# LouisRouss/DiffuLab

Hardware: AMD Instinct MI355X
Metric: train images/sec/node (DiT-S/2 flow-matching, 256x256 latents) (higher is better)
Workload: dtype bf16

## Files before the change

diffulab_amd/csrc/embed.hip:

```cpp
#include "common.h"
#include "aux_paths.h"
#include <atomic>

static std::atomic<int> g_last_aux_path{DL_AUX_PATH_NONE};
void dl_note_aux_path(int path) { g_last_aux_path.store(path, std::memory_order_relaxed); }
extern "C" __attribute__((visibility("default"))) int dl_lab_last_aux_path() { return g_last_aux_path.load(std::memory_order_relaxed); }

__global__ void patchify_k(const float* __restrict__ x, bf16_t* __restrict__ tok, int B, int C, int H, int W, int p,
                           int ld, int order) {
  const int gh = H / p, gw = W / p, F = C * p * p;
  const int64_t total = (int64_t)B * gh * gw * ld, stride = (int64_t)gridDim.x * blockDim.x;
  for (int64_t i = (int64_t)blockIdx.x * blockDim.x + threadIdx.x; i < total; i += stride) {
    const int f = (int)(i % ld);
    const int64_t t = i / ld;
    float val = 0.f;
    if (f < F) {
      const int wq = (int)(t % gw), hq = (int)((t / gw) % gh), b = (int)(t / ((int64_t)gw * gh));
      int c, p1, p2;
      if (order == DL_PATCH_CPP) {
        p2 = f % p;
        p1 = (f / p) % p;
        c = f / (p * p);
      } else {
        c = f % C;
// ... 148 lines not shown
                                     dl_stream_t stream) {
  DL_CHECK_ARG(t && out && B > 0 && dim > 0 && dim % 2 == 0, "dl_timestep_embedding: dim must be even");
  const int half = (int)(dim / 2);
  int64_t g = (B * half + 255) / 256;
  if (g > 1024) g = 1024;
  hipLaunchKernelGGL(timestep_embedding_k, (int)g, 256, 0, (hipStream_t)stream, t, (bf16_t*)out, (int)B, (int)dim,
                     (float)(-log((double)max_period) / (double)half));
  DL_LAUNCH_CHECK();
  return DL_OK;
}

__global__ void cond_combine_fwd_k(const float* __restrict__ e, const float* __restrict__ table,
                                   const int64_t* __restrict__ idx, float* __restrict__ emb, bf16_t* __restrict__ act,
                                   int B, int E) {
  const int64_t total = (int64_t)B * E;
  for (int64_t i = (int64_t)blockIdx.x * blockDim.x + threadIdx.x; i < total; i += (int64_t)gridDim.x * blockDim.x) {
    const int b = (int)(i / E), c = (int)(i % E);
    float v = e[i];
    if (idx) v += table[idx[b] * E + c];
    emb[i] = v;
    act[i] = f2bf(silu_f(v));
  }
}
extern "C" int dl_cond_combine_fwd(const float* e, const float* table, const int64_t* idx, float* emb, void* act,
                                   int64_t B, int64_t E, dl_stream_t stream) {
  DL_CHECK_ARG(e && emb && act && B > 0 && E > 0 && (!idx || table), "dl_cond_combine_fwd: bad args");
  int64_t g = (B * E + 255) / 256;
  if (g > 1024) g = 1024;
  hipLaunchKernelGGL(cond_combine_fwd_k, (int)g, 256, 0, (hipStream_t)stream, e, table, idx, emb, (bf16_t*)act, (int)B,
                     (int)E);
  DL_LAUNCH_CHECK();
  return DL_OK;
}
__global__ void cond_combine_bwd_k(const float* __restrict__ dact, const float* __restrict__ emb,
                                   const int64_t* __restrict__ idx, float* __restrict__ demb,
                                   bf16_t* __restrict__ demb16, float* __restrict__ dtable, int B, int E) {
  const int64_t total = (int64_t)B * E;
  for (int64_t i = (int64_t)blockIdx.x * blockDim.x + threadIdx.x; i < total; i += (int64_t)gridDim.x * blockDim.x) {
    const int b = (int)(i / E), c = (int)(i % E);
    const float g = dact[i] * dsilu_f(emb[i]);
    demb[i] = g;
    if (demb16) demb16[i] = f2bf(g);
    if (dtable && idx) {
      const int64_t lab = idx[b];
      bool first = true;
      for (int b2 = 0; b2 < b; ++b2) first = first && idx[b2] != lab;
      if (first) {
        float acc = g;
        for (int b2 = b + 1; b2 < B; ++b2)
          if (idx[b2] == lab) acc += dact[(int64_t)b2 * E + c] * dsilu_f(emb[(int64_t)b2 * E + c]);
        dtable[lab * E + c] += acc;
      }
    }
  }
}
extern "C" int dl_cond_combine_bwd(const float* dact, const float* emb, const int64_t* idx, float* demb, void* demb_bf16,
                                   float* dtable, int64_t B, int64_t E, dl_stream_t stream) {
  DL_CHECK_ARG(dact && emb && demb && B > 0 && E > 0, "dl_cond_combine_bwd: bad args");
  int64_t g = (B * E + 255) / 256;
  if (g > 1024) g = 1024;
  hipLaunchKernelGGL(cond_combine_bwd_k, (int)g, 256, 0, (hipStream_t)stream, dact, emb, idx, demb, (bf16_t*)demb_bf16,
                     dtable, (int)B, (int)E);
  DL_LAUNCH_CHECK();
  return DL_OK;
}

__global__ void cond_combine_dense_fwd_k(const float* __restrict__ e, const float* __restrict__ pe, float* __restrict__ emb,
                                         bf16_t* __restrict__ act, int64_t n4) {
  for (int64_t i = (int64_t)blockIdx.x * blockDim.x + threadIdx.x; i < n4; i += (int64_t)gridDim.x * blockDim.x) {
    const float4 a = ((const float4*)e)[i], p = ((const float4*)pe)[i];
    const float4 v = make_float4(a.x + p.x, a.y + p.y, a.z + p.z, a.w + p.w);
    ((float4*)emb)[i] = v;
    ((uint2*)act)[i] = make_uint2((uint32_t)f2bf(silu_f(v.x)) | ((uint32_t)f2bf(silu_f(v.y)) << 16),
                                  (uint32_t)f2bf(silu_f(v.z)) | ((uint32_t)f2bf(silu_f(v.w)) << 16));
  }
}
extern "C" int dl_cond_combine_dense_fwd(const float* e, const float* pe, float* emb, void* act, int64_t B, int64_t E,
                                         dl_stream_t stream) {
  DL_CHECK_ARG(e && pe && emb && act && B > 0 && E > 0 && E % 4 == 0 && ((uintptr_t)e | (uintptr_t)pe | (uintptr_t)emb) % 16 == 0 &&
                   (uintptr_t)act % 8 == 0,
               "dl_cond_combine_dense_fwd: contiguous [B, E] operands, E a multiple of 4 (E=%lld), f32 operands 16-byte, act 8-byte aligned",
               (long long)E);
  const int64_t n4 = B * E / 4;
  int64_t g = (n4 + 255) / 256;
  if (g > 1024) g = 1024;
  hipLaunchKernelGGL(cond_combine_dense_fwd_k, (int)g, 256, 0, (hipStream_t)stream, e, pe, emb, (bf16_t*)act, n4);
  DL_LAUNCH_CHECK();
  return DL_OK;
}
__global__ void cond_combine_dense_bwd_k(const float* __restrict__ dact, const float* __restrict__ emb, float* __restrict__ demb,
                                         bf16_t* __restrict__ demb16, int64_t n4) {
  for (int64_t i = (int64_t)blockIdx.x * blockDim.x + threadIdx.x; i < n4; i += (int64_t)gridDim.x * blockDim.x) {
    const float4 d = ((const float4*)dact)[i], v = ((const float4*)emb)[i];
    const float4 g = make_float4(d.x * dsilu_f(v.x), d.y * dsilu_f(v.y), d.z * dsilu_f(v.z), d.w * dsilu_f(v.w));
    ((float4*)demb)[i] = g;
// ... 459 lines not shown
```

diffulab_amd/engine.py:

```python

from __future__ import annotations

import functools
import math
from dataclasses import dataclass, field

import torch
from torch import Tensor

from . import ops, tuning


_PARAM_EPOCH = 0


def bump_param_epoch() -> None:
    global _PARAM_EPOCH
    _PARAM_EPOCH += 1


def _must(ok: bool) -> None:
    if not ok:
        raise RuntimeError("a HIP kernel declined a shape the engine had selected it for")


def _rup(x: int, m: int) -> int:
    return (x + m - 1) // m * m


STREAMS = ("input", "context")
ROW_MAX_DIM = 4096
F32_MAX_DIM = 1024


@functools.lru_cache(maxsize=None)
def block_names(pre: str, st: str | None = None) -> dict[str, str]:
    if st is None:
        n = dict(n1="norm_1", n2="norm_2", qk="attention.qk_norm", qkv="attention.qkv", proj="attention.proj_out", up="mlp_input.0",
                 down="mlp_input.2")
    else:
        n = dict(n1=f"{st}_norm_1", n2=f"{st}_norm_2", qk=f"attention.qk_norm_{st}", qkv=f"attention.qkv_{st}",
                 proj=f"attention.{st}_proj_out", up=f"mlp_{st}.0", down=f"mlp_{st}.2")
    return {k: pre + v for k, v in n.items()}


@dataclass(slots=True)
class Modulation:
    mat: Tensor
    dmat: Tensor | None
    off: int
    D: int
    rows: int
    tok: bool = False
    part: Tensor | tuple | None = None
    groups: int = 0

    def col(self, c: int) -> Tensor:
        o = self.off + c * self.D
        return self.mat[:, o : o + self.D]

# ... 474 lines not shown
        B, _, _, _, _, _, M, _, _ = self.geo
        D, E = d.inner_dim, d.embedding_dim
        ops.patchify(x, w["tokP"], d.patch_size, ops.PATCH_CPP)
        if patch_gemm:
            ops.gemm_nt(w["tokP"], sh[self._conv_name + "|f"], w["x"][0] if x0 is None else x0, M=M, N=D, K=self._ki)
        ops.timestep_embedding(t, w["temb"][:B])
        ops.gemm_nt(w["temb"], sh["time_embed.0.weight|f"], w["h1"], bias=self.P("time_embed.0.bias"), act=ops.ACT_SILU,
                    pre_out=w["pre1"], M=B, N=E, K=d.frequency_embedding)
        ops.gemm_nt(w["h1"], sh["time_embed.2.weight|f"], w["e"], bias=self.P("time_embed.2.bias"), M=B, N=E, K=E)
        if self._pooled_dim:
            self._pooled_fwd(B)
        else:
            table = self.P("label_embed.embedding.weight") if d.n_classes is not None else None
            ops.cond_combine_fwd(w["e"][:B], table, y_eff if table is not None else None, w["emb"][:B], w["se"][:B])
        mod_bias = self.params[self.layout.entries[self.layout.mod_b0][0] :][: self.layout.mod_rows]
        ops.gemm_nt(w["se"], sh["@mod|f"], w["mod"], bias=mod_bias, M=B, N=self.layout.mod_rows, K=E)
        return w["mod"]

    def _pooled_fwd(self, B: int) -> None:
        d, w, sh = self.d, self.ws, self.sh
        E, P = d.embedding_dim, self._pooled_dim
        pooled = self.pooled
        assert pooled is not None and tuple(pooled.shape) == (B, P), "pooled context embedding [B, pooled_dim] not set for this step"
        w["poolP"][:B, :P].copy_(pooled)
        ops.gemm_nt(w["poolP"], sh["mlp_pooled_context.0.weight|f"], w["ph1"], bias=self.P("mlp_pooled_context.0.bias"), act=ops.ACT_SILU,
                    pre_out=w["ppre1"], M=B, N=2 * E, K=w["poolP"].shape[1])
        ops.gemm_nt(w["ph1"], sh["mlp_pooled_context.2.weight|f"], w["pe"], bias=self.P("mlp_pooled_context.2.bias"), M=B, N=E, K=2 * E)
        ops.cond_combine_dense_fwd(w["e"][:B], w["pe"][:B], w["emb"][:B], w["se"][:B])

    def _pooled_bwd(self, B: int, det: Tensor | None) -> None:
        d, w, sh = self.d, self.ws, self.sh
        E, P = d.embedding_dim, self._pooled_dim
        ops.colsum(w["demb"], self.G("mlp_pooled_context.2.bias"), B, E, scratch=det)
        ops.gemm_tn(w["demb16"], w["ph1"], self.G("mlp_pooled_context.2.weight"), scratch=det)
        ops.gemm_nt(w["demb16"], sh["mlp_pooled_context.2.weight|t"], w["dph1"], M=B, N=2 * E, K=E)
        ops.silu_bwd(w["dph1"][:B], w["ppre1"][:B], w["dppre1"][:B])
        ops.gemm_tn(w["dppre1"], w["poolP"], self.G("mlp_pooled_context.0.weight"), M=2 * E, N=P, scratch=det)
        ops.colsum(w["dppre1"], self.G("mlp_pooled_context.0.bias"), B, 2 * E, scratch=det)

    def _main_wgs(self) -> int:
        explicit = tuning.integer("DL_MAIN_WGS", 0)
        if explicit:
            return explicit
        reserve = tuning.integer("DL_DP_RESERVE_CUS", 0)
        if reserve and self.reducer is not None and getattr(self.reducer, "enabled", True):
            if getattr(self, "_cus", None) is None:
                self._cus = torch.cuda.get_device_properties(self.dev).multi_processor_count
            return max(8, (self._cus - reserve) & ~7)
        return 0

    def _native_blocks(self) -> bool:
        return type(self) is DiTEngine and tuning.on("DL_NATIVE_BLOCK") and not (self.geo is not None and ops.attn_needs_padding(self.geo[5]))

    def _block_args(self, i: int, train: bool):
        key = (self._ws_key, i, self.reducer is None, self._main_wgs())
        blk = self._blk_cache.get(key)
        if blk is not None:
            return blk
        from ._block import DitBlock

        d, w, sh = self.d, self.ws, self.sh
        B, _, _, gh, gw, N, M, Bp, Fo = self.geo
        D, L, F = d.inner_dim, d.depth, d.mlp_ratio * d.inner_dim
        pre, mo = f"layers.{i}.", i * 6 * D
        mod, xs = w["mod"], w["x"]
        a = w["layers"][i if train else 0]
        xin = xs[i] if train else xs[i & 1]
        cos, sin = self._rope[(gh, gw)]
        mrow = lambda off: mod.data_ptr() + 2 * off
        blk = DitBlock()
        blk.B, blk.N, blk.D, blk.H, blk.F = B, N, D, d.num_heads, F
# ... 513 lines not shown
        _must(ops.ln_modulate_gemm_bwd(g["du"], sh[nm["up"] + ".weight|t"], a["x1"], self.P(nm["n2"] + ".weight"),
                                        self.P(nm["n2"] + ".bias"), mod[:, mo + 3 * D : mo + 4 * D], N, a["mean2"], a["rstd2"], dx, nx,
                                        dmod[:, mo + 3 * D : mo + 4 * D], dmod[:, mo + 4 * D : mo + 5 * D], w["dwb"][2 * i + 1],
                                        gate_t=a["t1"], gate=mod[:, mo + 2 * D : mo + 3 * D], dt=g["dt1"],
                                        dgate=dmod[:, mo + 2 * D : mo + 3 * D]))
        if fold:
            sw.fold(w["dwb"][2 * i + 1], nm["n2"] + ".weight", self.geo[0])
        dx = nx
        sw.wgrad(g["dt1"], a["a"], nm["proj"] + ".weight")
        ops.gemm_nt(g["dt1"], sh[nm["proj"] + ".weight|t"], s["da"])
        self._attn_bwd(a, g, nm, s, N, *self._rope[(gh, gw)], None, None, None)
        sw.wgrad(g["dqkv"], a["xm1"], nm["qkv"] + ".weight")
        if dres is not None:
            ops.add_bf16(dx, dres, dx)
        nxt = {}
        if i > 0:
            mp = (i - 1) * 6 * D
            nxt = dict(gate_t=w["layers"][i - 1]["t2"], gate=mod[:, mp + 5 * D : mp + 6 * D], dt=w["wg"][i - 1]["dt2"],
                       dgate=dmod[:, mp + 5 * D : mp + 6 * D])
        nx = _other(s, dx)
        _must(ops.ln_modulate_gemm_bwd(g["dqkv"], sh[nm["qkv"] + ".weight|t"], w["x"][i], self.P(nm["n1"] + ".weight"),
                                        self.P(nm["n1"] + ".bias"), mod[:, mo : mo + D], N, a["mean1"], a["rstd1"], dx, nx,
                                        dmod[:, mo : mo + D], dmod[:, mo + D : mo + 2 * D], w["dwb"][2 * i], **nxt))
        if fold:
            sw.fold(w["dwb"][2 * i], nm["n1"] + ".weight", self.geo[0])
        return nx

    def _head_bwd(self, dpred: Tensor, dxm: Tensor | None, scratch: Tensor | None = None) -> None:
        d, w = self.d, self.ws
        M, Fo, D = self.geo[6], self.geo[8], d.inner_dim
        ops.patchify(dpred, w["dO"], d.patch_size, ops.PATCH_PPC)
        gl = self.G("last_layer.linear.weight")
        if Fo % 8 == 0:
            ops.gemm_tn(w["dO"], w["xf"], gl, M=Fo, N=D, scratch=scratch)
        else:
            w["scr_last"].zero_()
            ops.gemm_tn(w["dO"], w["xf"], w["scr_last"], M=_rup(Fo, 8), N=D, scratch=scratch)
            ops.reduce_rows_f32(w["scr_last"], gl, 1, Fo * D)
        ops.colsum(w["dO"], self.G("last_layer.linear.bias"), M, Fo, scratch=scratch)
        if dxm is not None:
            ops.gemm_nt(w["dO"], self.sh["last_layer.linear.weight|t"], dxm, M=M, N=D, K=self._ko)

    def _dfeat_rows(self, dfeats: dict[int, Tensor] | None) -> dict[int, Tensor]:
        return {k: g.reshape(-1, self.d.inner_dim).to(torch.bfloat16).contiguous() for k, g in (dfeats or {}).items()}

    def _patch_wgrad(self, dx: Tensor, name: str, scratch: Tensor | None) -> None:
        d, w = self.d, self.ws
        D, Fi = d.inner_dim, d.input_channels * d.patch_size**2
        gc = self.G(name).view(D, Fi)
        if Fi % 8 == 0:
            ops.gemm_tn(dx, w["tokP"], gc, M=D, N=Fi, scratch=scratch)
        else:
            w["scr_conv"].zero_()
            ops.gemm_tn(dx, w["tokP"], w["scr_conv"], M=D, N=_rup(Fi, 8), scratch=scratch)
            gc.add_(w["scr_conv"][:, :Fi])

    def _end_block(self, sw: "SideWork", bi: int) -> None:
        sw.flush()
        if self.reducer is not None:
            self.reducer.ready(*self.layer_ranges[bi], extra_events=(sw.side.record_event(),))

    def _cond_bwd(self, dx: Tensor, extra_demb: Tensor | None = None) -> None:
        d, w, sh = self.d, self.ws, self.sh
        B, _, _, _, _, _, M, _, _ = self.geo
        D, E = d.inner_dim, d.embedding_dim
        dmod = w["dmod32"]
        det = w.get("det_scr")
        self._patch_wgrad(dx, self._conv_name, det)

        R = self.layout.mod_rows
        g_modw = self.grads[self.layout.entries[self.mod_name][0] :][: R * E].view(R, E)
        g_modb = self.grads[self.layout.entries[self.layout.mod_b0][0] :][:R]
        L6 = len(self.prefixes) * 6 * D if getattr(self, "_early_mod_done", False) else 0
        if L6:
            ops.cast2d_f32_to_bf16(dmod[:B, L6:], w["dmod"][:B, L6:])
            dmod = w["dmod"]
            ops.gemm_tn(dmod[:, L6:], w["se"], g_modw[L6:], scratch=det)
            ops.colsum(dmod[:, L6:], g_modb[L6:], B, R - L6, scratch=det)
        else:
            ops.cast_f32_to_bf16(dmod[:B], w["dmod"][:B])
            dmod = w["dmod"]
            ops.gemm_tn(dmod, w["se"], g_modw, scratch=det)
            ops.colsum(dmod, g_modb, B, R, scratch=det)
        ops.gemm_nt(dmod, sh["@mod|t"], w["dse"], M=B, N=E, K=R, scratch=det)
        table = d.n_classes is not None
        if self._pooled_dim:
            ops.cond_combine_dense_bwd(w["dse"][:B], w["emb"][:B], w["demb"][:B], w["demb16"][:B])
            self._pooled_bwd(B, det)
        else:
            ops.cond_combine_bwd(w["dse"][:B], w["emb"][:B], self._yeff if table else None, w["demb"][:B], w["demb16"][:B],
                                 self.G("label_embed.embedding.weight") if table else None)
        if extra_demb is not None:
            w["demb"][:B].add_(extra_demb[:B])
            ops.cast_f32_to_bf16(w["demb"][:B], w["demb16"][:B])
        ops.colsum(w["demb"], self.G("time_embed.2.bias"), B, E, scratch=det)
        ops.gemm_tn(w["demb16"], w["h1"], self.G("time_embed.2.weight"), scratch=det)
        ops.gemm_nt(w["demb16"], sh["time_embed.2.weight|t"], w["dh1"], M=B, N=E, K=E)
        ops.silu_bwd(w["dh1"][:B], w["pre1"][:B], w["dpre1"][:B])
        ops.gemm_tn(w["dpre1"], w["temb"], self.G("time_embed.0.weight"), scratch=det)
        ops.colsum(w["dpre1"], self.G("time_embed.0.bias"), B, E, scratch=det)
        if self.reducer is not None:
            if L6:
                w_mod = self.layout.entries[self.mod_name][0]
                self.reducer.ready(0, w_mod)
                self.reducer.ready(w_mod + L6 * E, self.layer_ranges[0][0])
            else:
                self.reducer.ready(0, self.layer_ranges[0][0])
            self.reducer.finish()


class _StrictWgradGroups(ops.WgradGroups):

    def _issue(self, key: int) -> None:
        probs = self.pending.pop(key, [])
        if probs:
            self.launch(lambda: _must(ops.gemm_tn_group(probs, self.slab, max_wgs=self.max_wgs)))


class _NoSideWork:

    def wgrad(self, dy: Tensor, x: Tensor, name: str) -> None:
        pass

    def fold(self, partial: Tensor | None, name: str, groups: int) -> None:
        pass

    def flush(self) -> None:
        pass

    def join(self) -> None:
        pass


# ... 35 lines not shown
```

diffulab_amd/ops.py:

```python

from __future__ import annotations

import ctypes
import os

import torch
from torch import Tensor

from ._lib import lib
from . import tuning

BF16, F32 = 0, 1
ACT_NONE, ACT_SILU, ACT_GELU = 0, 1, 2
LOSS_FLOW, LOSS_EPS = 0, 1
MEAN_TYPES = {"epsilon": 0, "xstart": 1, "xprev": 2, "v": 3}
VAR_MODES = {"learned": 0, "learned_range": 1}
VAR_FIXED = -1
PATCH_CPP, PATCH_PPC = 0, 1


_raw_stream = getattr(torch._C, "_cuda_getCurrentRawStream", None)


def _s() -> int:
# ... 539 lines not shown
    gemm_nt(dt, w2t, dh)
    swiglu_bwd(dh, u, du)


def mlp_dswiglu_recompute(x: Tensor, wp: Tensor, dt: Tensor, w2t: Tensor, du: Tensor) -> bool:
    M, F = x.shape[0], w2t.shape[0]
    return _maybe("dl_mlp_dswiglu_recompute", _p(x), x.stride(0), _p(wp), wp.stride(0), _p(dt), dt.stride(0), _p(w2t), w2t.stride(0),
                  _p(du), du.stride(0), M, F, x.shape[1], dt.shape[1], _s())


def _padded_rows(t: Tensor) -> Tensor:
    base = t._base
    if base is not None and base.dim() == t.dim() and base.shape[1:] == t.shape[1:] and base.data_ptr() == t.data_ptr() \
            and base.shape[0] == (t.shape[0] + 63) // 64 * 64 and base.stride() == t.stride():
        return base
    return t


def gemm_tn(a: Tensor, b: Tensor, out: Tensor, *, M: int | None = None, N: int | None = None, max_wgs: int = 0,
            scratch: Tensor | None = None) -> Tensor:
    M = a.shape[1] if M is None else M
    N = b.shape[1] if N is None else N
    if a.shape[0] % 64:
        a, b = _padded_rows(a), _padded_rows(b)
        assert a.shape[0] == b.shape[0], "gemm_tn operands with a ragged row count must be zero-padded row buffers"
    if scratch is not None:
        _call("dl_gemm_tn_det", _p(a), a.stride(0), _p(b), b.stride(0), _p(out), out.stride(0), M, N, a.shape[0], _p(scratch),
              scratch.numel(), _s())
        return out
    _call("dl_gemm_tn_ex", _p(a), a.stride(0), _p(b), b.stride(0), _p(out), out.stride(0), M, N, a.shape[0], int(max_wgs), _s())
    return out


class _WGrad(ctypes.Structure):

    _fields_ = [("dy", ctypes.c_void_p), ("ld_dy", ctypes.c_int64), ("x", ctypes.c_void_p), ("ld_x", ctypes.c_int64),
                ("g", ctypes.c_void_p), ("m_out", ctypes.c_int64), ("n_in", ctypes.c_int64)]


def gemm_tn_group(probs: list[tuple[Tensor, Tensor, Tensor]], slab: Tensor, max_wgs: int = 0) -> bool:
    arr = (_WGrad * len(probs))()
    if probs[0][0].shape[0] % 64:
        probs = [(_padded_rows(dy), _padded_rows(x), g) for dy, x, g in probs]
    R = probs[0][0].shape[0]
    for q, (dy, x, g) in zip(arr, probs):
        assert dy.shape[0] == R and x.shape[0] == R and g.is_contiguous()
        q.dy, q.ld_dy, q.x, q.ld_x, q.g, q.m_out, q.n_in = _p(dy), dy.stride(0), _p(x), x.stride(0), _p(g), g.shape[0], g.shape[1]
    global _LIB
    if _LIB is None:
        _LIB = lib()
    fn = _LIB._fns["dl_gemm_tn_group"][0]
    rc = fn(ctypes.addressof(arr), len(probs), R, _p(slab), slab.numel(), int(max_wgs), _s())
    if rc == -3:
        return False
    if rc != 0:
        raise RuntimeError(f"dl_gemm_tn_group failed ({rc}): {_LIB.cdll.dl_last_error().decode()}")
    return True


_SCRATCH: dict = {}


def shared_scratch(device, floats: int) -> Tensor:
    key = (torch.device(device).type, torch.device(device).index)
    buf = _SCRATCH.get(key)
    if buf is None or buf.numel() < floats:
# ... 980 lines not shown
```

diffulab_amd/tuning.py:

```python

from __future__ import annotations

import os

SWITCHES: dict[str, tuple[str, str]] = {
    "DL_NATIVE_BLOCK": ("1", "DiT blocks issued by the C ABI's block drivers (dl_dit_block_fwd / _bwd) instead of one Python call per kernel"),
    "DL_ROW_GEMM": ("1", "LayerNorm-modulate forward / backward as epilogues of the row-complete 256x384 GEMMs (D = 384, 256 tokens per sample)"),
    "DL_ROW_GEMM_QK": ("0", "QK-norm + RoPE as the epilogue of the qkv GEMM (measured slower than the separate row kernel)"),
    "DL_QKN_ON_LOAD": ("1", "QK-RMSNorm statistics leave with the qkv GEMM (dl_gemm_nt_ssq) and norm + RoPE are applied as the attention "
                       "forward stages q and k (dl_attn_fwd_qkn): no qk_norm_rope_fwd pass (row-complete path, <= 256 tokens)"),
    "DL_MLP_RECOMPUTE": ("1", "SwiGLU backward recomputes the MLP-up pre-activations instead of storing them in the forward"),
    "DL_ATTN_V_IN_PLACE": ("1", "attention reads V / writes dV inside the token-major qkv rows (N <= 256)"),
    "DL_QK_INPLACE": ("1", "attention backward writes dQ / dK token-major and the QK-norm backward runs in place on the dqkv rows"),
    "DL_WGRAD_GROUP": ("1", "the four weight gradients of a block as one atomics-free launch (dl_gemm_tn_group)"),
    "DL_WGRAD_INLINE": ("0", "grouped weight gradients on the main stream instead of the side stream"),
    "DL_WGRAD_SERIAL": ("0", "per-problem weight gradients on the main stream (engines without the grouped form)"),
    "DL_SIDE_WGS": ("", "workgroup cap of the side-stream weight gradients (default: 256 grouped, 128 per-problem)"),
    "DL_SIDE_CU_MASK": ("", "CU mask of the side stream (dl_stream_create_masked): 'i4' = every 4th CU, 'b128' = the first 128"),
    "DL_SIDE_LOW_PRIORITY": ("0", "DiT engines: the side stream of the weight gradients is created with the device's lowest stream priority "
                             "(measured +-0: DiT-S/2 20.83 / 20.80 vs 20.73 / 20.77 ms; SPRINT joint 28.77 / 28.58 vs 28.79 / 28.62; DDT 38.93 / 38.97 vs "
                             "39.01 / 39.00; joint MMDiT 49.14 / 49.13 vs 49.24 / 49.31; REPA 11.71 / 11.68 vs 11.76 / 11.73)"),
    "DL_UNET_SIDE_LOW_PRIORITY": ("1", "UNet: the same (the dispatcher serves the main chain's workgroups first: 26.42 / 26.50 vs 26.66 / 26.64 ms)"),
    "DL_JOIN_LAST": ("1", "single GPU: the side stream is joined after the conditioning backward instead of before it"),
    "DL_DP_RESERVE_CUS": ("0", "data parallel: CUs left to the communication library's workgroups (persistent main-chain grids shrink by it; "
                          "measured a loss at the headline shape, whose tile counts are whole multiples of 256: DESIGN.md section 5)"),
    "DL_MAIN_WGS": ("", "workgroup budget of the persistent main-chain kernels (experiments; default: all CUs, or CUs - reserve with a reducer)"),
    "DL_DP_EARLY_MOD": ("1", "data parallel: each block's adaLN rows are reduced as the block finishes"),
    "DL_HIPGRAPH": ("1", "samplers replay the denoiser forward as a captured hipGraph"),
    "DL_CFG_PAIR": ("1", "guided sampler steps run the conditional and the label-dropped forward as ONE forward over [x ; x] "
                    "(class-conditional MMDiT / DDT / UNetModel: same values per row, the weights stream once)"),
    "DL_LAUNCH_PLAN": ("0", "UNet (bf16 regime): a training forward / backward is recorded on its second run for a shape and re-issued as a "
                       "flat list of C calls afterwards (ops.LaunchPlan: the engine's Python costs the host ~24 us per launch, 716 "
                       "launches per step).  Measured (profiles/r06_e_*): the step at B = 64 is NOT host-bound -- its main queue is busy "
                       "19.2 of 20.3 ms and `host_issue` is the full launch queue pushing back -- so the plan changes nothing there "
                       "(20.03 vs 20.11 ms); it pays where the host is the slower side (under a profiler's per-launch overhead: 20.3 vs "
                       "22.7 ms), hence opt-in"),
    "DL_UNET_SIDE": ("1", "UNet weight gradients on a side stream"),
    "DL_UNET_NT_PAIR": ("1", "UNet AttentionBlock: the q and kv projections (and their data gradients) as one launch of the 128 x 128 GEMM "
                        "kernel where both are small (dl_gemm_nt_pair: 64 + 128 tiles on 256 CUs at the 4 x 4 level); bit-identical"),
    "DL_UNET_XATTN_HIP": ("1", "UNet TransformerBlock (context conditioning): the cross-attention core as dl_attn_cross_* (bf16 operands, f32 "
                          "softmax; MFMA with the keys streamed in 64-key tiles where dh % 64 == 0, VALU otherwise) where Nq <= 64, L <= 512, "
                          "dh % 8 == 0; 0 = the f32 copies + batched dl_f32_gemm + masked softmax fallback"),
    "DL_UNET_SPLITK": ("1", "split-K convolutions at the UNet's low-resolution levels (partial images + fixed-order fold: -7 % per step)"),
    "DL_UNET_WGRAD_WGS": ("128", "workgroup cap of the UNet's side-stream convolution weight gradients (0 = one per CU).  Round 6, with the "
                          "tap-reusing kernel and partial images (every workgroup stores its 295 KB of accumulators once, so the cap also "
                          "halves the stage bytes), B = 128: 0 -> 25.4 ms/step, 160 -> 24.1, 128 -> 23.9, 96 -> 24.4, 64 -> 25.0, 48 -> 26.8; "
                          "B = 64: 0 -> 19.0, 128 -> 18.0 (profiles/r06_q_*).  Round 5 (implicit-GEMM kernels, atomics): 0 was best"),
    "DL_UNET_FOLD_BATCHED": ("1", "UNet convolution weight gradients stay in a persistent transposed staging arena during the backward; one "
                             "launch at its end folds all of them into the [Co, Ci, 3, 3] gradients (instead of a zero-fill and a fold per convolution)"),
    "DL_UNET_WGRAD_PARTS": ("1", "UNet convolution weight gradients as partial images per pixel range (plain stores + fixed-order fold in the "
                            "batched fold launch: bit-reproducible) instead of f32 atomics into one image.  With the tap-reusing kernel of "
                            "round 6 (conv_wgrad.hip) the atomics were 56 % of a launch (1.45 TB/s of read-modify-writes against 6 TB/s of "
                            "stores) and the fold takes one tap of a channel tile per workgroup when eight or more images wait: B = 128 "
                            "24.7 -> 23.9 ms/step, B = 64 19.0 -> 18.0 (same workgroup cap).  With the implicit-GEMM kernels alone it was "
                            "slower (28.5 vs 26.8 ms: session e)"),
    "DL_UNET_DET_COLSUM": ("0", "UNet bias gradients through the bit-reproducible column sum (measured 2 % slower)"),
}


def text(name: str) -> str:
# ... 11 lines not shown
```

include/diffulab_hip.h:

```cpp
#ifndef DIFFULAB_HIP_H
#define DIFFULAB_HIP_H

#include <stdint.h>

#ifdef __cplusplus
extern "C" {
#endif

#define DL_API __attribute__((visibility("default")))

typedef void* dl_stream_t;

enum { DL_OK = 0, DL_ERR_INVALID = -1, DL_ERR_LAUNCH = -2, DL_ERR_UNSUPPORTED = -3 };
enum { DL_BF16 = 0, DL_F32 = 1 };
enum { DL_ACT_NONE = 0, DL_ACT_SILU = 1, DL_ACT_GELU = 2 };
enum { DL_LOSS_FLOW = 0, DL_LOSS_EPS = 1 };
enum { DL_MEAN_EPSILON = 0, DL_MEAN_XSTART = 1, DL_MEAN_XPREV = 2, DL_MEAN_V = 3 };
enum { DL_VAR_LEARNED = 0, DL_VAR_LEARNED_RANGE = 1 };
enum { DL_VAR_FIXED = -1 };
enum { DL_PATCH_CPP = 0, DL_PATCH_PPC = 1 };

DL_API int dl_version(void);
DL_API const char* dl_last_error(void);
DL_API int dl_device_info(int device, int* cu_count, int* lds_bytes_per_cu, int64_t* hbm_bytes, char* arch,
// ... 131 lines not shown
  void* C;
  int64_t ldc;
  int64_t M, N, K;
  const float* bias;
  const void* resid;
  int64_t ldr;
} dl_nt_problem_t;
DL_API int dl_gemm_nt_pair(const dl_nt_problem_t* problems, int n, dl_stream_t stream);
DL_API int dl_gemm_nt_swiglu(const void* X, int64_t ldx, const void* Wp, int64_t ldw, void* U, int64_t ldu, void* H,
                             int64_t ldh, int64_t M, int64_t F, int64_t K, dl_stream_t stream);
DL_API int dl_mlp_dswiglu_recompute(const void* X, int64_t ldx, const void* Wp, int64_t ldwp, const void* dT, int64_t ldt,
                                    const void* W2t, int64_t ldw2, void* dU, int64_t lddu, int64_t M, int64_t F, int64_t K1,
                                    int64_t K2, dl_stream_t stream);
DL_API int dl_gemm_tn(const void* A, int64_t lda, const void* B, int64_t ldb, float* C, int64_t ldc, int64_t M,
                      int64_t N, int64_t R, dl_stream_t stream);
DL_API int dl_gemm_tn_ex(const void* A, int64_t lda, const void* B, int64_t ldb, float* C, int64_t ldc, int64_t M,
                         int64_t N, int64_t R, int max_workgroups, dl_stream_t stream);
typedef struct dl_wgrad_t {
  const void* dy;
  int64_t ld_dy;
  const void* x;
  int64_t ld_x;
  float* g;
  int64_t m_out, n_in;
} dl_wgrad_t;
DL_API int dl_gemm_tn_group(const dl_wgrad_t* probs, int n_probs, int64_t R, float* slab, int64_t slab_floats, int max_workgroups,
                            dl_stream_t stream);
DL_API int dl_gemm_tn_det(const void* A, int64_t lda, const void* B, int64_t ldb, float* C, int64_t ldc, int64_t M, int64_t N,
                          int64_t R, float* scratch, int64_t scratch_floats, dl_stream_t stream);
DL_API int dl_gemm_nt_f32_det(const void* A, int64_t lda, const void* B, int64_t ldb, float* C, int64_t ldc, int64_t M, int64_t N,
                              int64_t K, float* scratch, int64_t scratch_floats, dl_stream_t stream);
DL_API int dl_colsum_det(const void* x, int dtype, int64_t ld, float* out, int64_t R, int64_t C, float* scratch,
                         int64_t scratch_floats, dl_stream_t stream);

DL_API int dl_ln_modulate_fwd(const void* x, const float* w, const float* b, const void* scale, const void* shift,
                              int64_t ld_mod, int64_t rows_per_mod, float eps, void* out, float* mean,
                              float* rstd, const void* t, const void* gate, int64_t ld_gate, void* x_out, int64_t M,
                              int64_t D, dl_stream_t stream);
DL_API int dl_ln_modulate_bwd(const void* dout, const void* x, const float* w, const float* b, const void* scale,
                              int64_t ld_mod, int64_t rows_per_mod, const float* mean, const float* rstd,
                              const void* dres, void* dx, float* dscale, float* dshift, int64_t ld_dmod,
                              float* dwb_partial, const void* gate_t, const void* gate, int64_t ld_gate, void* dt,
                              float* dgate, int64_t M, int64_t D, dl_stream_t stream);
DL_API int dl_ln_modulate_bwd_tok(const void* dout, const void* x, const float* w, const float* b, const void* scale,
                                  int64_t ld_mod, const float* mean, const float* rstd, const void* dres, void* dx, void* dscale,
                                  void* dshift, int64_t ld_dmod, float* dwb_partial, int64_t n_part, const void* gate_t,
                                  const void* gate, int64_t ld_gate, void* dt, void* dgate, int64_t M, int64_t D,
                                  dl_stream_t stream);
DL_API int dl_ln_modulate_gemm_fwd(const void* A, int64_t lda, const void* W, int64_t ldw, int64_t M, int64_t K, const void* resid,
                                   const void* gate, int64_t ld_gate, const float* ln_w, const float* ln_b, const void* scale,
                                   const void* shift, int64_t ld_mod, int64_t rows_per_mod, float eps, void* t_out, void* x_out,
                                   void* xm_out, float* mean, float* rstd, int64_t D, dl_stream_t stream);
DL_API int dl_ln_modulate_gemm_bwd(const void* A, int64_t lda, const void* Wt, int64_t ldw, int64_t M, int64_t K, const void* x,
                                   const float* ln_w, const float* ln_b, const void* scale, int64_t ld_mod, int64_t rows_per_mod,
                                   const float* mean, const float* rstd, const void* dres, void* dx, float* dscale, float* dshift,
                                   int64_t ld_dmod, float* dwb_partial, const void* gate_t, const void* gate, int64_t ld_gate,
                                   void* dt, float* dgate, int64_t D, dl_stream_t stream);
DL_API int dl_gemm_nt_qk_norm_rope(const void* A, int64_t lda, const void* Wqkv, int64_t ldw, int64_t B, int64_t N, int64_t H,
                                   int64_t dh, int64_t rot, float eps, const float* scale_q, const float* scale_k, const float* cos,
                                   const float* sin, void* qkv, void* q, void* k, float* rrms, int64_t n_dst, int64_t n_off,
                                   dl_stream_t stream);
DL_API int dl_ddt_cond_fwd(const void* enc, int64_t ld, const float* temb, int64_t ld_t, int64_t B, int64_t N, int64_t D, void* out,
                           dl_stream_t stream);
DL_API int dl_ddt_cond_bwd(const void* dsz, const void* enc, int64_t ld, const float* temb, int64_t ld_t, int64_t B, int64_t N,
                           int64_t D, void* denc, float* dtemb, dl_stream_t stream);
DL_API int dl_gate_bwd(const void* dout, const void* t, const void* gate, int64_t ld_mod, int64_t rows_per_mod,
// ... 362 lines not shown
```

Before: 12460.

## Add skinny weight-gradient GEMM kernels and stage class-label dedup in LDS

Adds two specialized TN GEMM kernels: a short-reduction kernel that fuses the f32-to-bf16 cast, the weight-gradient product, the bias column sum and the bf16 copy for the adaLN, time-embedding and pooled MLP weight gradients, and a tall-reduction split-K kernel for the last-layer and patch-embedding weight gradients. These replace separate cast, deterministic GEMM and colsum launches, cutting launches and extra passes over the activations. The class-embedding backward now stages labels in LDS and precomputes a per-label linked list, replacing the quadratic global scans. Both paths are gated by a new DL_SKINNY flag that defaults on, and each falls back to the old path when the shape does not fit. The risk is that results may differ from the deterministic path in summation order.

```diff
diff --git a/diffulab_amd/csrc/embed.hip b/diffulab_amd/csrc/embed.hip
--- a/diffulab_amd/csrc/embed.hip
+++ b/diffulab_amd/csrc/embed.hip
@@ -204,9 +204,28 @@
   DL_LAUNCH_CHECK();
   return DL_OK;
 }
+#define COND_LDS_LABELS 2048
+template <bool STAGED>
 __global__ void cond_combine_bwd_k(const float* __restrict__ dact, const float* __restrict__ emb,
                                    const int64_t* __restrict__ idx, float* __restrict__ demb,
                                    bf16_t* __restrict__ demb16, float* __restrict__ dtable, int B, int E) {
+  __shared__ int64_t s_idx[STAGED ? COND_LDS_LABELS : 1];
+  __shared__ int s_next[STAGED ? COND_LDS_LABELS : 1];
+  if (STAGED) {
+    for (int b = threadIdx.x; b < B; b += blockDim.x) s_idx[b] = idx[b];
+    __syncthreads();
+    for (int b = threadIdx.x; b < B; b += blockDim.x) {
+      const int64_t lab = s_idx[b];
+      int earlier = 0, nx = B;
+#pragma unroll 8
+      for (int b2 = 0; b2 < b; ++b2) earlier += s_idx[b2] == lab;
+#pragma unroll 8
+      for (int b2 = b + 1; b2 < B; ++b2) nx = min(nx, s_idx[b2] == lab ? b2 : B);
+      nx = nx < B ? nx : -1;
+      s_next[b] = earlier == 0 ? nx : -2 - (nx + 1);
+    }
+    __syncthreads();
+  }
   const int64_t total = (int64_t)B * E;
   for (int64_t i = (int64_t)blockIdx.x * blockDim.x + threadIdx.x; i < total; i += (int64_t)gridDim.x * blockDim.x) {
     const int b = (int)(i / E), c = (int)(i % E);
@@ -214,6 +233,19 @@
     demb[i] = g;
     if (demb16) demb16[i] = f2bf(g);
     if (dtable && idx) {
+      if (STAGED) {
+        int nx = s_next[b];
+        if (nx >= -1) {
+          float acc = g;
+          while (nx >= 0) {
+            acc += dact[(int64_t)nx * E + c] * dsilu_f(emb[(int64_t)nx * E + c]);
+            const int e = s_next[nx];
+            nx = -2 - e - 1;
+          }
+          dtable[s_idx[b] * E + c] += acc;
+        }
+        continue;
+      }
       const int64_t lab = idx[b];
       bool first = true;
       for (int b2 = 0; b2 < b; ++b2) first = first && idx[b2] != lab;
@@ -231,8 +263,12 @@
   DL_CHECK_ARG(dact && emb && demb && B > 0 && E > 0, "dl_cond_combine_bwd: bad args");
   int64_t g = (B * E + 255) / 256;
   if (g > 1024) g = 1024;
-  hipLaunchKernelGGL(cond_combine_bwd_k, (int)g, 256, 0, (hipStream_t)stream, dact, emb, idx, demb, (bf16_t*)demb_bf16,
-                     dtable, (int)B, (int)E);
+  if (dtable && idx && B <= COND_LDS_LABELS)
+    hipLaunchKernelGGL(cond_combine_bwd_k<true>, (int)g, 256, 0, (hipStream_t)stream, dact, emb, idx, demb, (bf16_t*)demb_bf16,
+                       dtable, (int)B, (int)E);
+  else
+    hipLaunchKernelGGL(cond_combine_bwd_k<false>, (int)g, 256, 0, (hipStream_t)stream, dact, emb, idx, demb, (bf16_t*)demb_bf16,
+                       dtable, (int)B, (int)E);
   DL_LAUNCH_CHECK();
   return DL_OK;
 }
diff --git a/diffulab_amd/csrc/gemm_skinny.hip b/diffulab_amd/csrc/gemm_skinny.hip
--- /dev/null
+++ b/diffulab_amd/csrc/gemm_skinny.hip
@@ -0,0 +1,298 @@
+#include "common.h"
+
+int launch_fold_partials(const float* part, int64_t stride, int splits, int64_t M, int64_t N, int64_t ldp, float* C, int64_t ldc,
+                         int accumulate, hipStream_t stream);
+
+typedef __attribute__((address_space(3))) s16x4_t lds_s16x4_t;
+
+template <int COLS>
+__device__ __forceinline__ int sk_slot_off(int r, int q) {
+  return r * (COLS * 2) + ((q ^ ((r & 3) << 2)) << 4);
+}
+template <int COLS>
+__device__ __forceinline__ bf16x8_t sk_frag(const char* tile, int col0, int kk, int lane) {
+  const int li = lane & 15, g = lane >> 4;
+  const int col = col0 + (g & 1) * 16 + (li & 3) * 4;
+  const int r0 = kk * 16 + (g >> 1) * 8 + (li >> 2);
+  union {
+    s16x4_t h[2];
+    bf16x8_t v;
+  } u;
+  u.h[0] = __builtin_amdgcn_ds_read_tr16_b64_v4i16((lds_s16x4_t*)(tile + sk_slot_off<COLS>(r0, col >> 3) + (col & 7) * 2));
+  u.h[1] = __builtin_amdgcn_ds_read_tr16_b64_v4i16((lds_s16x4_t*)(tile + sk_slot_off<COLS>(r0 + 4, col >> 3) + (col & 7) * 2));
+  return u.v;
+}
+__device__ __forceinline__ u32x4_t sk_round8(const f32x4_t& x, const f32x4_t& y) {
+  return u32x4_t{pack2bf(x[0], x[1]), pack2bf(x[2], x[3]), pack2bf(y[0], y[1]), pack2bf(y[2], y[3])};
+}
+
+template <bool AF32>
+struct SkRegs {
+  f32x4_t xa[AF32 ? 2 : 1][2];
+  u32x4_t ra[AF32 ? 1 : 2], rb[2];
+};
+template <bool AF32>
+__global__ __launch_bounds__(256, 3) void gemm_tn_short_k(const void* __restrict__ A_, int64_t lda, const bf16_t* __restrict__ Bm,
+                                                           int64_t ldb, float* __restrict__ C, int64_t ldc, int M, int N, int R,
+                                                           int accumulate, float* __restrict__ csum, bf16_t* __restrict__ acopy,
+                                                           int64_t ldcp) {
+  extern __shared__ __attribute__((aligned(16))) char smem[];
+  const int tiles_n = (N + 127) / 128, tiles_m = (M + 127) / 128;
+  const int lid = xcd_remap((int)blockIdx.x, tiles_m * tiles_n);
+  const int m0 = (lid / tiles_n) * 128, n0 = (lid % tiles_n) * 128;
+  const bool side = (lid % tiles_n) == 0;
+  const int t = threadIdx.x, lane = t & 63;
+  const int wave = __builtin_amdgcn_readfirstlane(t >> 6);
+  const int wr = wave >> 1, wc = wave & 1;
+
+  const int q = t & 15, rg = t >> 4;
+  const int cm = m0 + q * 8, cn = n0 + q * 8;
+  const bool va = cm + 8 <= M;
+  const int cmc = va ? cm : M - 8;
+  const int cnc = cn + 8 <= N ? cn : N - 8;
+  const int woff = sk_slot_off<128>(rg, q);
+  auto load = [&](int st, SkRegs<AF32>& g) {
+#pragma unroll
+    for (int c = 0; c < 2; ++c) {
+      const int row = st * 32 + rg + 16 * c;
+      if (AF32) {
+        const float* p = (const float*)A_ + (int64_t)row * lda + cmc;
+        g.xa[AF32 ? c : 0][0] = *(const f32x4_t*)p;
+        g.xa[AF32 ? c : 0][1] = *(const f32x4_t*)(p + 4);
+      } else {
+        g.ra[AF32 ? 0 : c] = *(const u32x4_t*)((const bf16_t*)A_ + (int64_t)row * lda + cmc);
+      }
+      g.rb[c] = *(const u32x4_t*)(Bm + (int64_t)row * ldb + cnc);
+    }
+  };
+  float cs[8];
+#pragma unroll
+  for (int e = 0; e < 8; ++e) cs[e] = 0.f;
+  auto store = [&](int st, int buf, const SkRegs<AF32>& g) {
+    char* ba = smem + buf * 16384 + woff;
+    char* bb = ba + 8192;
+#pragma unroll
+    for (int c = 0; c < 2; ++c) {
+      const u32x4_t pa = AF32 ? sk_round8(g.xa[AF32 ? c : 0][0], g.xa[AF32 ? c : 0][1]) : g.ra[AF32 ? 0 : c];
+      *(u32x4_t*)(ba + c * 4096) = pa;
+      *(u32x4_t*)(bb + c * 4096) = g.rb[c];
+      if (side) {
+        if (csum) {
+          float f[8];
+          unpack8(pa, f);
+#pragma unroll
+          for (int e = 0; e < 8; ++e) cs[e] += f[e];
+        }
+        if (AF32 && acopy && va) *(u32x4_t*)(acopy + (int64_t)(st * 32 + rg + 16 * c) * ldcp + cm) = pa;
+      }
+    }
+  };
+
+  f32x16_t acc[2][2];
+#pragma unroll
+  for (int i = 0; i < 2; ++i)
+#pragma unroll
+    for (int j = 0; j < 2; ++j)
+#pragma unroll
+      for (int r = 0; r < 16; ++r) acc[i][j][r] = 0.f;
+  auto multiply = [&](int buf) {
+    const char* ta = smem + buf * 16384;
+    const char* tb = ta + 8192;
+#pragma unroll
+    for (int kk = 0; kk < 2; ++kk) {
+      bf16x8_t af[2], bfg[2];
+#pragma unroll
+      for (int i = 0; i < 2; ++i) {
+        af[i] = sk_frag<128>(ta, wr * 64 + i * 32, kk, lane);
+        bfg[i] = sk_frag<128>(tb, wc * 64 + i * 32, kk, lane);
+      }
+#pragma unroll
+      for (int i = 0; i < 2; ++i)
+#pragma unroll
+        for (int j = 0; j < 2; ++j) acc[i][j] = __builtin_amdgcn_mfma_f32_32x32x16_bf16(af[i], bfg[j], acc[i][j], 0, 0, 0);
+    }
+  };
+
+  const int nst = R / 32;
+  SkRegs<AF32> g0, g1;
+  load(0, g0);
+  if (nst > 1) load(1, g1);
+  for (int st = 0; st < nst; st += 2) {
+    store(st, 0, g0);
+    __syncthreads();
+    if (st + 2 < nst) load(st + 2, g0);
+    multiply(0);
+    if (st + 1 < nst) {
+      store(st + 1, 1, g1);
+      __syncthreads();
+      if (st + 3 < nst) load(st + 3, g1);
+      multiply(1);
+    }
+  }
+
+  if (side && csum) {
+    __syncthreads();
+    float* red = (float*)smem;
+#pragma unroll
+    for (int e = 0; e < 8; ++e) red[rg * 128 + q * 8 + e] = cs[e];
+    __syncthreads();
+    if (t < 128 && m0 + t < M) {
+      float s = 0.f;
+#pragma unroll
+      for (int g = 0; g < 16; ++g) s += red[g * 128 + t];
+      csum[m0 + t] = accumulate ? csum[m0 + t] + s : s;
+    }
+  }
+
+#pragma unroll
+  for (int i = 0; i < 2; ++i) {
+    float old[2][16];
+#pragma unroll
+    for (int j = 0; j < 2; ++j) {
+      const int n = n0 + wc * 64 + j * 32 + (lane & 31);
+#pragma unroll
+      for (int r = 0; r < 16; ++r) {
+        const int m = m0 + wr * 64 + i * 32 + (r & 3) + 8 * (r >> 2) + 4 * (lane >> 5);
+        old[j][r] = (accumulate && m < M && n < N) ? C[(int64_t)m * ldc + n] : 0.f;
+      }
+    }
+#pragma unroll
+    for (int j = 0; j < 2; ++j) {
+      const int n = n0 + wc * 64 + j * 32 + (lane & 31);
+#pragma unroll
+      for (int r = 0; r < 16; ++r) {
+        const int m = m0 + wr * 64 + i * 32 + (r & 3) + 8 * (r >> 2) + 4 * (lane >> 5);
+        if (m < M && n < N) C[(int64_t)m * ldc + n] = accumulate ? old[j][r] + acc[i][j][r] : acc[i][j][r];
+      }
+    }
+  }
+}
+
+#define TL_STAGE (64 * 768 + 64 * 256)
+template <bool WIDE_M>
+__global__ __launch_bounds__(256, 1) void gemm_tn_tall_k(const bf16_t* __restrict__ Wd, int64_t ldw, const bf16_t* __restrict__ Nr,
+                                                          int64_t ldn, int narrow, int nchunks, float* __restrict__ part) {
+  extern __shared__ __attribute__((aligned(16))) char smem[];
+  const int s = blockIdx.x, S = gridDim.x;
+  const int c_lo = (int)((int64_t)nchunks * s / S), c_hi = (int)((int64_t)nchunks * (s + 1) / S);
+  const int t = threadIdx.x, lane = t & 63;
+  const int wave = __builtin_amdgcn_readfirstlane(t >> 6);
+
+  const int nrow = t >> 2, nq = t & 3;
+  const int ncol = nq * 8 + 8 <= narrow ? nq * 8 : narrow - 8;
+  u32x4_t rw[12], rn;
+  auto load = [&](int ch) {
+    const int64_t r0 = (int64_t)ch * 64;
+#pragma unroll
+    for (int c = 0; c < 12; ++c) {
+      const int it = t + 256 * c;
+      const int row = it / 48, sl = it - row * 48;
+      rw[c] = *(const u32x4_t*)(Wd + (r0 + row) * ldw + sl * 8);
+    }
+    rn = *(const u32x4_t*)(Nr + (r0 + nrow) * ldn + ncol);
+  };
+  auto store = [&](int buf) {
+    char* bw = smem + buf * TL_STAGE;
+    char* bn = bw + 64 * 768;
+#pragma unroll
+    for (int c = 0; c < 12; ++c) {
+      const int it = t + 256 * c;
+      const int row = it / 48, sl = it - row * 48;
+      *(u32x4_t*)(bw + sk_slot_off<384>(row, sl)) = rw[c];
+    }
+    *(u32x4_t*)(bn + sk_slot_off<128>(nrow, nq)) = rn;
+  };
+
+  f32x16_t acc[3];
+#pragma unroll
+  for (int j = 0; j < 3; ++j)
+#pragma unroll
+    for (int r = 0; r < 16; ++r) acc[j][r] = 0.f;
+
+  if (c_lo < c_hi) load(c_lo);
+  for (int ch = c_lo; ch < c_hi; ++ch) {
+    const int buf = (ch - c_lo) & 1;
+    store(buf);
+    __syncthreads();
+    if (ch + 1 < c_hi) load(ch + 1);
+    const char* tw = smem + buf * TL_STAGE;
+    const char* tn = tw + 64 * 768;
+#pragma unroll
+    for (int kk = 0; kk < 4; ++kk) {
+      const bf16x8_t fn = sk_frag<128>(tn, 0, kk, lane);
+      bf16x8_t fw[3];
+#pragma unroll
+      for (int j = 0; j < 3; ++j) fw[j] = sk_frag<384>(tw, wave * 96 + j * 32, kk, lane);
+#pragma unroll
+      for (int j = 0; j < 3; ++j)
+        acc[j] = WIDE_M ? __builtin_amdgcn_mfma_f32_32x32x16_bf16(fw[j], fn, acc[j], 0, 0, 0)
+                        : __builtin_amdgcn_mfma_f32_32x32x16_bf16(fn, fw[j], acc[j], 0, 0, 0);
+    }
+  }
+
+  float* img = part + (int64_t)s * narrow * 384;
+#pragma unroll
+  for (int j = 0; j < 3; ++j) {
+    const int colw = wave * 96 + j * 32;
+#pragma unroll
+    for (int r = 0; r < 16; ++r) {
+      const int row = (r & 3) + 8 * (r >> 2) + 4 * (lane >> 5), col = lane & 31;
+      if (WIDE_M) {
+        if (col < narrow) img[(int64_t)(colw + row) * narrow + col] = acc[j][r];
+      } else {
+        if (row < narrow) img[(int64_t)row * 384 + colw + col] = acc[j][r];
+      }
+    }
+  }
+}
+
+extern "C" int dl_gemm_tn_short(const void* A, int a_dtype, int64_t lda, const void* B, int64_t ldb, float* C, int64_t ldc, int64_t M,
+                                int64_t N, int64_t R, int accumulate, float* colsum, void* a_bf16, int64_t ld_a_bf16,
+                                dl_stream_t stream) {
+  DL_CHECK_ARG(A && B && C && M > 0 && N > 0 && R > 0, "dl_gemm_tn_short: null/empty operand");
+  DL_CHECK_ARG(a_dtype == DL_BF16 || a_dtype == DL_F32, "dl_gemm_tn_short: a_dtype %d", a_dtype);
+  if (R < 64 || R > 512 || R % 32 || N % 64 || M % 8) return DL_ERR_UNSUPPORTED;
+  DL_CHECK_ARG(lda % 8 == 0 && ldb % 8 == 0 && lda >= M && ldb >= N && ldc >= N && M < (1ll << 24) && N < (1ll << 24),
+               "dl_gemm_tn_short: leading dims (lda=%lld ldb=%lld ldc=%lld)", (long long)lda, (long long)ldb, (long long)ldc);
+  DL_CHECK_ARG((((uintptr_t)A | (uintptr_t)B) & 15) == 0 && ((uintptr_t)C & 3) == 0, "dl_gemm_tn_short: 16-byte alignment");
+  DL_CHECK_ARG(!a_bf16 || (a_dtype == DL_F32 && ld_a_bf16 % 8 == 0 && ld_a_bf16 >= M && ((uintptr_t)a_bf16 & 15) == 0),
+               "dl_gemm_tn_short: the bf16 copy needs an f32 A, ld %% 8 == 0 and 16-byte alignment");
+  const int64_t ntile = ((M + 127) / 128) * ((N + 127) / 128);
+  DL_CHECK_ARG(ntile < (1ll << 30), "dl_gemm_tn_short: too many tiles");
+  if (a_dtype == DL_F32)
+    hipLaunchKernelGGL(gemm_tn_short_k<true>, (int)ntile, 256, 32768, (hipStream_t)stream, A, lda, (const bf16_t*)B, ldb, C, ldc, (int)M,
+                       (int)N, (int)R, accumulate, colsum, (bf16_t*)a_bf16, ld_a_bf16);
+  else
+    hipLaunchKernelGGL(gemm_tn_short_k<false>, (int)ntile, 256, 32768, (hipStream_t)stream, A, lda, (const bf16_t*)B, ldb, C, ldc, (int)M,
+                       (int)N, (int)R, accumulate, colsum, (bf16_t*)nullptr, (int64_t)0);
+  DL_LAUNCH_CHECK();
+  return DL_OK;
+}
+
+extern "C" int dl_gemm_tn_tall(const void* A, int64_t lda, const void* B, int64_t ldb, float* C, int64_t ldc, int64_t M, int64_t N,
+                               int64_t R, float* scratch, int64_t scratch_floats, dl_stream_t stream) {
+  DL_CHECK_ARG(A && B && C && scratch && M > 0 && N > 0 && R > 0, "dl_gemm_tn_tall: null/empty operand");
+  const bool wide_m = M == 384 && (N == 16 || N == 32), wide_n = N == 384 && (M == 16 || M == 32);
+  if (!(wide_m || wide_n) || R % 64 || R < 2048 || R >= (1ll << 31)) return DL_ERR_UNSUPPORTED;
+  DL_CHECK_ARG(lda % 8 == 0 && ldb % 8 == 0 && lda >= M && ldb >= N && ldc >= N, "dl_gemm_tn_tall: leading dims (lda=%lld ldb=%lld ldc=%lld)",
+               (long long)lda, (long long)ldb, (long long)ldc);
+  DL_CHECK_ARG((((uintptr_t)A | (uintptr_t)B) & 15) == 0, "dl_gemm_tn_tall: 16-byte alignment");
+  DL_CHECK_ARG(scratch_floats >= M * N, "dl_gemm_tn_tall: scratch of %lld floats < one [M, N] image", (long long)scratch_floats);
+  static DevOnce once;
+  const int n_cu = dev_cus(once, [] {
+    (void)hipFuncSetAttribute((const void*)gemm_tn_tall_k<true>, hipFuncAttributeMaxDynamicSharedMemorySize, 2 * TL_STAGE);
+    (void)hipFuncSetAttribute((const void*)gemm_tn_tall_k<false>, hipFuncAttributeMaxDynamicSharedMemorySize, 2 * TL_STAGE);
+  });
+  const int nchunks = (int)(R / 64);
+  int64_t S = n_cu;
+  if (S > nchunks) S = nchunks;
+  if (S > scratch_floats / (M * N)) S = scratch_floats / (M * N);
+  if (wide_m)
+    hipLaunchKernelGGL(gemm_tn_tall_k<true>, (int)S, 256, 2 * TL_STAGE, (hipStream_t)stream, (const bf16_t*)A, lda, (const bf16_t*)B, ldb,
+                       (int)N, nchunks, scratch);
+  else
+    hipLaunchKernelGGL(gemm_tn_tall_k<false>, (int)S, 256, 2 * TL_STAGE, (hipStream_t)stream, (const bf16_t*)B, ldb, (const bf16_t*)A, lda,
+                       (int)M, nchunks, scratch);
+  DL_LAUNCH_CHECK();
+  return launch_fold_partials(scratch, M * N, (int)S, M, N, N, C, ldc, 1, (hipStream_t)stream);
+}
diff --git a/diffulab_amd/engine.py b/diffulab_amd/engine.py
--- a/diffulab_amd/engine.py
+++ b/diffulab_amd/engine.py
@@ -26,6 +26,12 @@
 
 def _rup(x: int, m: int) -> int:
     return (x + m - 1) // m * m
+
+
+def _short_wgrad(B: int, a: Tensor, b: Tensor, out: Tensor, colsum: Tensor | None = None, a_bf16: Tensor | None = None) -> bool:
+    if not tuning.on("DL_SKINNY") or B % 32 or b.shape[0] < B:
+        return False
+    return ops.gemm_tn_short(a[:B], b[:B], out, colsum=colsum, a_bf16=a_bf16)
 
 
 STREAMS = ("input", "context")
@@ -566,11 +572,14 @@
         d, w, sh = self.d, self.ws, self.sh
         E, P = d.embedding_dim, self._pooled_dim
         ops.colsum(w["demb"], self.G("mlp_pooled_context.2.bias"), B, E, scratch=det)
-        ops.gemm_tn(w["demb16"], w["ph1"], self.G("mlp_pooled_context.2.weight"), scratch=det)
+        if not _short_wgrad(B, w["demb16"], w["ph1"], self.G("mlp_pooled_context.2.weight")):
+            ops.gemm_tn(w["demb16"], w["ph1"], self.G("mlp_pooled_context.2.weight"), scratch=det)
         ops.gemm_nt(w["demb16"], sh["mlp_pooled_context.2.weight|t"], w["dph1"], M=B, N=2 * E, K=E)
         ops.silu_bwd(w["dph1"][:B], w["ppre1"][:B], w["dppre1"][:B])
-        ops.gemm_tn(w["dppre1"], w["poolP"], self.G("mlp_pooled_context.0.weight"), M=2 * E, N=P, scratch=det)
-        ops.colsum(w["dppre1"], self.G("mlp_pooled_context.0.bias"), B, 2 * E, scratch=det)
+        if not (w["poolP"].shape[1] == P and _short_wgrad(B, w["dppre1"], w["poolP"], self.G("mlp_pooled_context.0.weight"),
+                                                          colsum=self.G("mlp_pooled_context.0.bias"))):
+            ops.gemm_tn(w["dppre1"], w["poolP"], self.G("mlp_pooled_context.0.weight"), M=2 * E, N=P, scratch=det)
+            ops.colsum(w["dppre1"], self.G("mlp_pooled_context.0.bias"), B, 2 * E, scratch=det)
 
     def _main_wgs(self) -> int:
         explicit = tuning.integer("DL_MAIN_WGS", 0)
@@ -1150,7 +1159,8 @@
         ops.patchify(dpred, w["dO"], d.patch_size, ops.PATCH_PPC)
         gl = self.G("last_layer.linear.weight")
         if Fo % 8 == 0:
-            ops.gemm_tn(w["dO"], w["xf"], gl, M=Fo, N=D, scratch=scratch)
+            if not (scratch is not None and tuning.on("DL_SKINNY") and ops.gemm_tn_tall(w["dO"], w["xf"], gl, scratch, M=Fo, N=D)):
+                ops.gemm_tn(w["dO"], w["xf"], gl, M=Fo, N=D, scratch=scratch)
         else:
             w["scr_last"].zero_()
             ops.gemm_tn(w["dO"], w["xf"], w["scr_last"], M=_rup(Fo, 8), N=D, scratch=scratch)
@@ -1167,7 +1177,8 @@
         D, Fi = d.inner_dim, d.input_channels * d.patch_size**2
         gc = self.G(name).view(D, Fi)
         if Fi % 8 == 0:
-            ops.gemm_tn(dx, w["tokP"], gc, M=D, N=Fi, scratch=scratch)
+            if not (scratch is not None and tuning.on("DL_SKINNY") and ops.gemm_tn_tall(dx, w["tokP"], gc, scratch, M=D, N=Fi)):
+                ops.gemm_tn(dx, w["tokP"], gc, M=D, N=Fi, scratch=scratch)
         else:
             w["scr_conv"].zero_()
             ops.gemm_tn(dx, w["tokP"], w["scr_conv"], M=D, N=_rup(Fi, 8), scratch=scratch)
@@ -1191,15 +1202,17 @@
         g_modb = self.grads[self.layout.entries[self.layout.mod_b0][0] :][:R]
         L6 = len(self.prefixes) * 6 * D if getattr(self, "_early_mod_done", False) else 0
         if L6:
-            ops.cast2d_f32_to_bf16(dmod[:B, L6:], w["dmod"][:B, L6:])
+            if not _short_wgrad(B, dmod[:, L6:], w["se"], g_modw[L6:], colsum=g_modb[L6:], a_bf16=w["dmod"][:B, L6:]):
+                ops.cast2d_f32_to_bf16(dmod[:B, L6:], w["dmod"][:B, L6:])
+                ops.gemm_tn(w["dmod"][:, L6:], w["se"], g_modw[L6:], scratch=det)
+                ops.colsum(w["dmod"][:, L6:], g_modb[L6:], B, R - L6, scratch=det)
             dmod = w["dmod"]
-            ops.gemm_tn(dmod[:, L6:], w["se"], g_modw[L6:], scratch=det)
-            ops.colsum(dmod[:, L6:], g_modb[L6:], B, R - L6, scratch=det)
         else:
-            ops.cast_f32_to_bf16(dmod[:B], w["dmod"][:B])
+            if not _short_wgrad(B, dmod, w["se"], g_modw, colsum=g_modb, a_bf16=w["dmod"][:B]):
+                ops.cast_f32_to_bf16(dmod[:B], w["dmod"][:B])
+                ops.gemm_tn(w["dmod"], w["se"], g_modw, scratch=det)
+                ops.colsum(w["dmod"], g_modb, B, R, scratch=det)
             dmod = w["dmod"]
-            ops.gemm_tn(dmod, w["se"], g_modw, scratch=det)
-            ops.colsum(dmod, g_modb, B, R, scratch=det)
         ops.gemm_nt(dmod, sh["@mod|t"], w["dse"], M=B, N=E, K=R, scratch=det)
         table = d.n_classes is not None
         if self._pooled_dim:
@@ -1212,11 +1225,13 @@
             w["demb"][:B].add_(extra_demb[:B])
             ops.cast_f32_to_bf16(w["demb"][:B], w["demb16"][:B])
         ops.colsum(w["demb"], self.G("time_embed.2.bias"), B, E, scratch=det)
-        ops.gemm_tn(w["demb16"], w["h1"], self.G("time_embed.2.weight"), scratch=det)
+        if not _short_wgrad(B, w["demb16"], w["h1"], self.G("time_embed.2.weight")):
+            ops.gemm_tn(w["demb16"], w["h1"], self.G("time_embed.2.weight"), scratch=det)
         ops.gemm_nt(w["demb16"], sh["time_embed.2.weight|t"], w["dh1"], M=B, N=E, K=E)
         ops.silu_bwd(w["dh1"][:B], w["pre1"][:B], w["dpre1"][:B])
-        ops.gemm_tn(w["dpre1"], w["temb"], self.G("time_embed.0.weight"), scratch=det)
-        ops.colsum(w["dpre1"], self.G("time_embed.0.bias"), B, E, scratch=det)
+        if not _short_wgrad(B, w["dpre1"], w["temb"], self.G("time_embed.0.weight"), colsum=self.G("time_embed.0.bias")):
+            ops.gemm_tn(w["dpre1"], w["temb"], self.G("time_embed.0.weight"), scratch=det)
+            ops.colsum(w["dpre1"], self.G("time_embed.0.bias"), B, E, scratch=det)
         if self.reducer is not None:
             if L6:
                 w_mod = self.layout.entries[self.mod_name][0]
diff --git a/diffulab_amd/ops.py b/diffulab_amd/ops.py
--- a/diffulab_amd/ops.py
+++ b/diffulab_amd/ops.py
@@ -595,6 +595,25 @@
     return out
 
 
+def gemm_tn_short(a: Tensor, b: Tensor, out: Tensor, *, accumulate: bool = True, colsum: Tensor | None = None,
+                  a_bf16: Tensor | None = None) -> bool:
+    R, M = a.shape
+    assert b.shape[0] == R and a.stride(1) == 1 and b.stride(1) == 1 and out.stride(1) == 1 and tuple(out.shape) == (M, b.shape[1])
+    assert colsum is None or (colsum.is_contiguous() and colsum.numel() == M)
+    assert a_bf16 is None or (tuple(a_bf16.shape) == (R, M) and a_bf16.stride(1) == 1)
+    return _maybe("dl_gemm_tn_short", _p(a), F32 if a.dtype == torch.float32 else BF16, a.stride(0), _p(b), b.stride(0), _p(out),
+                  out.stride(0), M, b.shape[1], R, int(accumulate), _p(colsum), _p(a_bf16), a_bf16.stride(0) if a_bf16 is not None else 0,
+                  _s())
+
+
+def gemm_tn_tall(a: Tensor, b: Tensor, out: Tensor, scratch: Tensor, *, M: int | None = None, N: int | None = None) -> bool:
+    M = a.shape[1] if M is None else M
+    N = b.shape[1] if N is None else N
+    assert a.shape[0] == b.shape[0]
+    return _maybe("dl_gemm_tn_tall", _p(a), a.stride(0), _p(b), b.stride(0), _p(out), out.stride(0), M, N, a.shape[0], _p(scratch),
+                  scratch.numel(), _s())
+
+
 class _WGrad(ctypes.Structure):
 
     _fields_ = [("dy", ctypes.c_void_p), ("ld_dy", ctypes.c_int64), ("x", ctypes.c_void_p), ("ld_x", ctypes.c_int64),
diff --git a/diffulab_amd/tuning.py b/diffulab_amd/tuning.py
--- a/diffulab_amd/tuning.py
+++ b/diffulab_amd/tuning.py
@@ -26,6 +26,9 @@
                           "measured a loss at the headline shape, whose tile counts are whole multiples of 256: DESIGN.md section 5)"),
     "DL_MAIN_WGS": ("", "workgroup budget of the persistent main-chain kernels (experiments; default: all CUs, or CUs - reserve with a reducer)"),
     "DL_DP_EARLY_MOD": ("1", "data parallel: each block's adaLN rows are reduced as the block finishes"),
+    "DL_SKINNY": ("1", "weight gradients outside the blocks through the one-pass skinny kernels where they take the shape: adaLN "
+                       "modulation linear (cast, product, bias gradient and bf16 copy in one launch), time / pooled-context MLPs "
+                       "(dl_gemm_tn_short), last layer and patch embedding (dl_gemm_tn_tall); 0 = dl_gemm_tn_det and its folds everywhere"),
     "DL_HIPGRAPH": ("1", "samplers replay the denoiser forward as a captured hipGraph"),
     "DL_CFG_PAIR": ("1", "guided sampler steps run the conditional and the label-dropped forward as ONE forward over [x ; x] "
                     "(class-conditional MMDiT / DDT / UNetModel: same values per row, the weights stream once)"),
diff --git a/include/diffulab_hip.h b/include/diffulab_hip.h
--- a/include/diffulab_hip.h
+++ b/include/diffulab_hip.h
@@ -187,6 +187,10 @@
                               int64_t K, float* scratch, int64_t scratch_floats, dl_stream_t stream);
 DL_API int dl_colsum_det(const void* x, int dtype, int64_t ld, float* out, int64_t R, int64_t C, float* scratch,
                          int64_t scratch_floats, dl_stream_t stream);
+DL_API int dl_gemm_tn_short(const void* A, int a_dtype, int64_t lda, const void* B, int64_t ldb, float* C, int64_t ldc, int64_t M,
+                            int64_t N, int64_t R, int accumulate, float* colsum, void* a_bf16, int64_t ld_a_bf16, dl_stream_t stream);
+DL_API int dl_gemm_tn_tall(const void* A, int64_t lda, const void* B, int64_t ldb, float* C, int64_t ldc, int64_t M, int64_t N,
+                           int64_t R, float* scratch, int64_t scratch_floats, dl_stream_t stream);
 
 DL_API int dl_ln_modulate_fwd(const void* x, const float* w, const float* b, const void* scale, const void* shift,
                               int64_t ld_mod, int64_t rows_per_mod, float eps, void* out, float* mean,
```

Measured after the change: 12520 (median of 6 runs). About the same (+0.6%).
